# sony/DiffRoll

Measured on AMD Instinct MI355X. Metric: piano-roll frames/sec (200-step sample), higher is better.
Workload: dtype f32

## Files before the change

diffroll_amd/csrc/abi.hip:

```cpp
#include "engine_state.h"
#include "tenants.h"

#include <algorithm>
#include <condition_variable>
#include <mutex>

namespace drh {

thread_local std::string g_create_error;
void release_stager(int dev);
std::atomic<int> g_engines[MAX_DEVICES];

struct FusedSlot {
    std::mutex mu;
    std::condition_variable cv;
    dr_engine* owner = nullptr;
    bool claimed = false;
    hipEvent_t done = nullptr;
};
FusedSlot g_slots[MAX_DEVICES];

bool claim_fused_slot(dr_engine* e, hipStream_t st) {
    FusedSlot& s = g_slots[e->cfg.device];
    std::unique_lock<std::mutex> lk(s.mu);
// ... 367 lines not shown
        (void)hipDeviceSynchronize();
        e->opt.solver = value;
        e->hist_key.valid = false;
        if (!e->committed) return DR_OK;
        return build_solver(e);
    }
    if (n == "solver_noise") {
        if (value != 0 && value != 1)
            return fail(e, DR_EINVAL, "solver_noise is 0 (the deterministic solver) or 1 (its stochastic form, SDE-DPM-Solver++), got %d", value);
        if (e->opt.solver_noise == value) return DR_OK;
        if (e->opt.solver != 0) (void)hipDeviceSynchronize();
        e->opt.solver_noise = value;
        e->hist_key.valid = false;
        if (!e->committed || e->opt.solver == 0) return DR_OK;
        return build_solver(e);
    }
    if (n == "start_step") {
        if (value < -1 || value >= e->S)
            return fail(e, DR_EINVAL, "start_step is -1 (the chain's first step) or in [0, timesteps = %d), got %d", e->S, value);
        e->opt.start = value;
        return DR_OK;
    }
    if (n == "start_noise") {
        if (value != 0 && value != 1)
            return fail(e, DR_EINVAL, "start_noise is 0 (x on entry is x at the start step) or 1 (a clean roll, diffused to it), got %d", value);
        e->opt.start_noise = value;
        return DR_OK;
    }
    if (n == "x0_clip") {
        if (value < 0 || value > 2)
            return fail(e, DR_EINVAL, "x0_clip is 0 (off), 1 (clamp the x0 prediction to [0, 1]) or 2 (to [-1, 1]), got %d", value);
        if (e->opt.x0_clamp != value) e->hist_key.valid = false;
        e->opt.x0_clamp = value;
        return DR_OK;
    }
    if (n == "x0_threshold") {
        if (value != 0 && (value < 5000 || value > 10000))
            return fail(e, DR_EINVAL, "x0_threshold is 0 (off) or the percentile in units of 1 / 10000, 5000 .. 10000 (9950 = 99.5 %%), got %d", value);
        if (e->opt.x0_thresh != value) e->hist_key.valid = false;
        e->opt.x0_thresh = value;
        return DR_OK;
    }
    if (n == "guidance_t_min" || n == "guidance_t_max") {
        const bool is_max = n == "guidance_t_max";
        if (!guidance_value_ok(is_max, value, e->S))
            return fail(e, DR_EINVAL, is_max ? "guidance_t_max is -1 (= timesteps - 1) or in [0, timesteps = %d), got %d"
                                             : "guidance_t_min is in [0, timesteps = %d), got %d", e->S, value);
        (is_max ? e->opt.guid.hi : e->opt.guid.lo) = value;
        return DR_OK;
    }
    if (!lab) return fail(e, DR_ENAME, "unknown option '%s'", name);
    if (n == "fused_stack_xcd") { if (e->opt_stack_xcd != value) drop(); e->opt_stack_xcd = value; return DR_OK; }
    if (n == "fused_stack_warm") { if (e->opt_stack_warm != value) drop(); e->opt_stack_warm = value; return DR_OK; }
#ifdef DR_FAULT_HOOK
    if (n == "stack_fault_test") { if (e->opt_stack_fault != value) drop(); e->opt_stack_fault = value; return DR_OK; }
#endif
    if (n == "stack_ticks") { if (e->stack_dbg_on != value) drop(); e->stack_dbg_on = value; return DR_OK; }
    if (n.compare(0, 5, "tune.") == 0) {
        Tuning& t = tuning();
        const std::string f = n.substr(5);
        if (f == "ksplit_blocks") {
            if (t.ksplit_blocks.load() != value) { t.ksplit_blocks.store(value); tuning_epoch().fetch_add(1); drop(); }
            return DR_OK;
        }
        std::atomic<int>* field = f == "pack_threads" ? &t.pack_threads : f == "tile" ? &t.tile : f == "pw" ? &t.pw : f == "pw_nw" ? &t.pw_nw
                   : f == "pwk" ? &t.pwk : f == "ksplit_max" ? &t.ksplit_max : f == "one_ks" ? &t.one_ks : f == "stack3" ? &t.stack3
                   : f == "stack_fl" ? &t.stack_fl : f == "tail_t4" ? &t.tail_t4 : f == "xcd_n" ? &t.xcd_n : f == "xcd_model" ? &t.xcd_model
                   : f == "s3_eager" ? &t.s3_eager : f == "debug_chunks" ? &t.debug_chunks : nullptr;
        if (!field) return fail(e, DR_ENAME, "unknown option '%s'", name);
        if (field->load() != value) {
            field->store(value);
            tuning_epoch().fetch_add(1);
            drop();
        }
        return DR_OK;
    }
    return fail(e, DR_ENAME, "unknown option '%s'", name);
}

int open_chain_call(dr_engine* e, int sampler, int B, int T, const int* step, int& NB, int& i0, hipStream_t st) {
    int rc = check_ready(e, sampler, B, T);
    if (rc) return rc;
    if (step) {
        const int t = *step;
        if (t < 0 || t >= e->S) return fail(e, DR_EINVAL, "step %d out of range", t);
        if (!e->rs_steps.empty() && std::find(e->rs_steps.begin(), e->rs_steps.end(), t) == e->rs_steps.end())
            return fail(e, DR_EINVAL, "step %d is not visited by the respaced chain (option sampling_steps = %d)", t, e->opt.steps);
    }
    if ((rc = check_options(e, sampler, B, NB, T))) return rc;
    i0 = 0;
    if (!step && (rc = start_position(e, i0))) return rc;
    if ((rc = ensure_workspace(e, NB, T))) return rc;
    if (e->opt.solver == 2) {
        const size_t need = 2 * (size_t)B * T * 88;
        if (!e->hist.fits(need)) e->hist_key.valid = false;
        if ((rc = grow_chain_buffer(e, e->hist, need, st))) return rc;
    }
    if (e->opt.x0_thresh != 0 && (rc = grow_chain_buffer(e, e->thresh_work, thresh_work_words(B), st))) return rc;
    return DR_OK;
}

}
using namespace drh;

extern "C" {

// ... 483 lines not shown
```

diffroll_amd/csrc/engine_state.h:

```cpp
#pragma once
#include <hip/hip_runtime.h>

#include <dlfcn.h>

#include <atomic>
#include <chrono>
#include <cmath>
#include <cstdarg>
#include <cstdio>
#include <cstdlib>
#include <cstring>
#include <map>
#include <memory>
#include <string>
#include <thread>
#include <vector>

#include "../../include/diffroll_amd_debug.h"
#include "device_buffer.h"
#include "fused_mode.h"
#include "kernels.h"

namespace drh {
using namespace dr;
// ... 95 lines not shown
    dr_config cfg{};
    int C = 0, Cp = 0, L = 0, K = 0, S = 0, NM = 0;
    int max_dil = 1;
    int n_bins = 0, bins_p = 0;
    std::string err;
    std::map<std::string, std::vector<float>> params;
    std::vector<float> h_emb, h_coef;
    std::vector<float> h_win, h_fb;
    float h_win_norm = 0.f;
    bool committed = false;

    drh::DevBuf<float> d_coef;
    drh::DevBuf<float> d_dtab;
    std::vector<drh::LayerW> layers;
    float *in_w = nullptr, *in_b = nullptr, *skip_w = nullptr, *skip_b = nullptr, *outp_w = nullptr, *outp_b = nullptr;
    float *dft_w = nullptr, *mel_w = nullptr;
    float *fft_win = nullptr, *fft_tw = nullptr;
    float fft_norm = 1.f;
    bool use_fft = false;
    std::vector<drh::DevBuf<float>> consts;

    int ws_NB = 0, ws_T = 0;
    drh::DevBuf<float> sk_ws;
    drh::DevBuf<unsigned> sk_cnt;
    drh::DevBuf<float> h, hd, g, skip, tmp, x0buf;
    drh::DevBuf<float> xwork;
    drh::DevBuf<float> hd3, g3;
    int prec = 0;
    bool s3_ready = false;
    double t_pack_s = 0.0, t_upload_s = 0.0, t_tables_s = 0.0, t_capture_s = 0.0;
    int norm_framewise = 0;
    int fe_B = 0, fe_T = 0;
    drh::DevBuf<float> cond;
    drh::DevBuf<float> cond_dummy;
    drh::DevBuf<float> cond_tr;
    int cond_tr_T = 0;
    drh::DevBuf<float> wav_pad, power, logmel, specP4, mm;

    drh::GraphKey gkey;
    hipGraph_t graph = nullptr;
    hipGraphExec_t gexec = nullptr;
    drh::DevBuf<long long> dbg_ticks;
    drh::DevBuf<unsigned long long> d_counts;
    size_t mm_scratch_off = 0;
    hipStream_t cap_stream = nullptr;
    drh::DevBuf<dr::DynParams> d_dyn;
    drh::DevBuf<int> d_tsel;
    bool use_dyn = false;

    drh::FusedMode fused;
    int opt_stack_xcd = 1;
    int opt_stack_fault = 0;
    int opt_stack_warm = 0;
    int n_cus = 0;
    drh::StackSync sync;
    int opt_tail = 1;
    int64_t tail_launches = 0;
    drh::ChainOptions opt;
    std::vector<int> win_marks;
    drh::DevBuf<unsigned> d_wintab;
    std::vector<int> rs_steps;
    drh::DevBuf<float> d_coef_rs;
    std::vector<float> h_solver;
    drh::DevBuf<float> d_solver;
    drh::DevBuf<float> hist;
    int hist_par = 0;
    struct { bool valid = false; int sampler = -1, B = 0, T = 0, t = -1; } hist_key;
    drh::DevBuf<unsigned> thresh_work;
    int64_t inproj_launches = 0;
    int64_t conv0_launches = 0;
    unsigned win_epoch = 0;
    drh::DevBuf<float> xalt;
    int last_mode = 0;
    unsigned tuning_epoch = 0;
    long kfd_gpu_id = -1;
    double last_tenant_scan_s = -1.0;
    hipStream_t graph_stream = nullptr;
    bool graph_stream_set = false;
    bool unverified = false;
    hipStream_t fused_stream = nullptr;
    int opt_blocked = 2;
    drh::DevBuf<float> xsave;
    drh::DevBuf<long long> stack_dbg;
    int stack_dbg_on = 0;
    int64_t stack_launches = 0;

    double prof_flops = 0.0;
    std::string prof_name;
    bool prof = false;
    std::vector<std::pair<hipEvent_t, hipEvent_t>> prof_events;
    size_t prof_used = 0;
    int64_t prof_launches = 0;
    double prof_ms = 0.0;

    ~dr_engine() {
        if (gexec) (void)hipGraphExecDestroy(gexec);
        if (graph) (void)hipGraphDestroy(graph);
        if (cap_stream) (void)hipStreamDestroy(cap_stream);
        for (auto& p : prof_events) { (void)hipEventDestroy(p.first); (void)hipEventDestroy(p.second); }
    }
};

namespace drh {

inline int fail(dr_engine* e, int code, const char* fmt, ...) {
    char buf[512];
// ... 103 lines not shown
```

diffroll_amd/csrc/gemm_body.h:

```cpp
#pragma once
#include "device_common.h"

namespace dr {

DR_DEVINL void residual_quad(const float (&v)[4], const float4 bias, const float4 prev, float (&o)[4]) {
    float bb[4], pv[4];
    f4arr(bias, bb); f4arr(prev, pv);
#pragma unroll
    for (int e = 0; e < 4; ++e) o[e] = div_sqrt2(pv[e] + (v[e] + bb[e]));
}
DR_DEVINL void skip_quad(const float (&v)[4], const float4 bias, const float4 prev, const bool skip_init, float (&o)[4]) {
    float bb[4], pv[4];
    f4arr(bias, bb); f4arr(prev, pv);
#pragma unroll
    for (int e = 0; e < 4; ++e) o[e] = skip_init ? v[e] + bb[e] : (v[e] + bb[e]) + pv[e];
}
DR_DEVINL long cond_row(const GemmArgs& a, const int b) {
    int r = a.c_b0 + b;
    if (a.c_n > 0 && r >= a.c_n) r %= a.c_n;
    return r;
}
DR_DEVINL void gate_quad(const float (&v0)[4], const float (&v1)[4], const float4 bias0, const float4 bias1,
                         const float4 cond0, const float4 cond1, const bool has_c, float (&o)[4]) {
    float b0[4], b1[4], c0[4], c1[4];
// ... 473 lines not shown
    #pragma unroll
                        for (int e = 0; e < 4; ++e) o[e] = v0[e] * v0[e] + v1[e] * v1[e];
                    }
                    if (a.out_s3 & 1) {
                        store_s3_quad<COH>(a.Y + (long)be * a.y_bs, o, c0, t, a.T, a.y_rows >> 3, a.wt_store);
                    } else {
                        float* dst = a.Y + (long)be * a.y_bs + (long)(c0 >> 2) * a.y_ps + (long)t * a.y_fs;
                        store_f4<COH>(dst, make_float4(o[0], o[1], o[2], o[3]), a.wt_store);
                    }
                } else {
                    const int p0 = mt * 128 + wave * 32 + rq;
                    float v[4], o[4];
    #pragma unroll
                    for (int e = 0; e < 4; ++e) v[e] = acc[ni][4 * q + e];
                    if constexpr (EPI == EPI_RES_SKIP) {
                        if (p0 < a.y_rows) {
                            float* dst = a.Y + (long)be * a.y_bs + (long)(p0 >> 2) * a.y_ps + (long)t * a.y_fs;
                            residual_quad(v, ebias[q], eop[ni][q], o);
                            *reinterpret_cast<float4*>(dst) = make_float4(o[0], o[1], o[2], o[3]);
                            if (a.Y2) store_y2<COH, 0>(a, be, o, ed2[q], p0, t);
                        } else {
                            float* dst = a.skip + (long)be * a.s_bs + ((long)((p0 - a.y_rows) >> 2) * a.T + t) * 4;
                            skip_quad(v, ebias[q], eop[ni][q], a.skip_init, o);
                            *reinterpret_cast<float4*>(dst) = make_float4(o[0], o[1], o[2], o[3]);
                        }
                    } else {
                        if (p0 >= a.y_rows) continue;
                        float bb[4];
                        f4arr(ebias[q], bb);
    #pragma unroll
                        for (int e = 0; e < 4; ++e) {
                            if constexpr (EPI == EPI_PLAIN) o[e] = a.alpha * v[e] + bb[e];
                            else if constexpr (EPI == EPI_RELU) o[e] = fmaxf(a.alpha * v[e] + bb[e], 0.f);
                            else if constexpr (EPI == EPI_SILU) { const float z = v[e] + bb[e]; o[e] = z * sigmoidf_(z); }
                            else o[e] = logf(v[e] + 1e-6f);
                        }
                        float* dst = a.Y + (long)be * a.y_bs + (long)(p0 >> 2) * a.y_ps + (long)t * a.y_fs;
                        *reinterpret_cast<float4*>(dst) = make_float4(o[0], o[1], o[2], o[3]);
                        if constexpr (EPI == EPI_RELU) {
                            if (a.Y2) store_y2<COH, 0>(a, be, o, ed2[q], p0, t);
                        }
                    }
                }
            }
        }
    }
    if (a.dbg && blockIdx.x == 0 && tid == 0) {
        a.dbg[0] = tick1 - tick0;
        a.dbg[1] = clock64() - tick0;
    }
}

template <int NW, int COH, int RLDS, int TBN = 32 * NW, int EPI = EPI_RES_SKIP>
DR_DEVINL void pw_body(const GemmArgs& a, const int mt, const int nt, const int wave, float4* Rs = nullptr, const int foff = 0) {
    static_assert(EPI == EPI_RES_SKIP || EPI == EPI_RELU || EPI == EPI_PLAIN, "pw_body epilogues");
    static_assert(EPI == EPI_RES_SKIP || !RLDS, "the LDS-resident tile belongs to the residual / skip epilogue");
    constexpr int BN = TBN;
    int lane = threadIdx.x & 63;
    if constexpr (COH) asm volatile("" : "+v"(lane));
    const int r = lane & 31, hi = lane >> 5;
    const long long tick0 = a.dbg ? clock64() : 0;

    const int tps = (a.T + BN - 1) / BN;
    const int b = nt / tps;
    const int t0 = (nt % tps) * BN + foff;
    const int NS = a.kchunks;

    const __amdgpu_buffer_rsrc_t wr = __builtin_amdgcn_make_buffer_rsrc(
        (void*)(a.Wp + (long)mt * NS * 4096), 0, (unsigned)NS * 16384u, 0x00020000);
    const __amdgpu_buffer_rsrc_t xr = __builtin_amdgcn_make_buffer_rsrc(
        (void*)(a.X + (long)b * a.x_bs), 0, (unsigned)(a.x_planes * a.x_ps * 4), 0x00020000);
    const int wvo = (hi * 128 + wave * 32 + r) * 16;
    const int xps = (int)a.x_ps * 4;
    int xvo[NW];
#pragma unroll
    for (int ni = 0; ni < NW; ++ni) xvo[ni] = hi * xps + min(t0 + ni * 32 + r, a.T - 1) * 16;

    struct BF { float4 v[4][NW]; };
    auto load_a = [&](int slab) { return load_a4(wr, wvo, slab, NS, 120); };
    auto load_b = [&](int slab) -> BF {
        BF o;
#pragma unroll
        for (int g = 0; g < 4; ++g)
#pragma unroll
            for (int ni = 0; ni < NW; ++ni)
                o.v[g][ni] = buffer_load_f4(xr, xvo[ni], (slab * 8 + g * 2) * xps);
        return o;
    };

    f32x16 acc[NW];
#pragma unroll
    for (int ni = 0; ni < NW; ++ni)
#pragma unroll
        for (int e = 0; e < 16; ++e) acc[ni][e] = 0.f;

    AF4 aA = load_a(0), aB;
    BF bA = load_b(0), bB;
    auto step = [&](auto ROLE, int slab) {
        constexpr bool kB = decltype(ROLE)::value;
        const int nxt = min(slab + 1, NS - 1);
        if constexpr (kB) { aA = load_a(nxt); bA = load_b(nxt); }
        else { aB = load_a(nxt); bB = load_b(nxt); }
#pragma unroll
        for (int g = 0; g < 4; ++g) {
            const float4 af = kB ? aB.v[g] : aA.v[g];
#pragma unroll
            for (int ni = 0; ni < NW; ++ni) acc[ni] = __builtin_amdgcn_mfma_f32_32x32x2f32(af.x, (kB ? bB.v[g][ni] : bA.v[g][ni]).x, acc[ni], 0, 0, 0);
// ... 22 lines not shown
        const float* base = res_rows ? a.Y + (long)b * a.y_bs + (long)(rowb >> 2) * a.y_ps
                                     : a.skip + (long)b * a.s_bs + (long)((rowb - a.y_rows) >> 2) * a.T * 4;
        const long qs = res_rows ? 2 * a.y_ps : (long)2 * a.T * 4;
        const long fs = res_rows ? a.y_fs : 4;
#pragma unroll
        for (int ni = 0; ni < NW; ++ni) {
            const int tc = min(t0 + ni * 32 + r, a.T - 1);
#pragma unroll
            for (int q = 0; q < 4; ++q) eop[ni][q] = *reinterpret_cast<const float4*>(base + q * qs + tc * fs);
        }
    };
    int slab = 0;
    const int pre = max(NS - 2, 0) & ~1;
    for (; slab < pre; slab += 2) {
        step(std::false_type{}, slab);
        step(std::true_type{}, slab + 1);
        if (a.dbg && slab == 0 && blockIdx.x == 0 && threadIdx.x == 0) a.dbg[2] = clock64() - tick0;
    }
    if (a.dbg && blockIdx.x == 0 && threadIdx.x == 0) a.dbg[3] = clock64() - tick0;
    if constexpr (!RLDS) load_epilogue();
    __builtin_amdgcn_sched_barrier(0);
    for (; slab + 2 <= NS; slab += 2) {
        step(std::false_type{}, slab);
        step(std::true_type{}, slab + 1);
    }
    if (slab < NS) step(std::false_type{}, slab);
    const long long tick1 = a.dbg ? clock64() : 0;
    if constexpr (RLDS) load_epilogue();

#pragma unroll
    for (int ni = 0; ni < NW; ++ni) {
        const int t = t0 + ni * 32 + r;
        if (t >= a.T) continue;
#pragma unroll
        for (int q = 0; q < 4; ++q) {
            const int p0 = rowb + 8 * q;
            float v[4], o[4];
#pragma unroll
            for (int e = 0; e < 4; ++e) v[e] = acc[ni][4 * q + e];
            if constexpr (EPI != EPI_RES_SKIP) {
                if (p0 >= a.y_rows) continue;
                float bb[4];
                f4arr(ebias[q], bb);
#pragma unroll
                for (int e = 0; e < 4; ++e) {
                    o[e] = a.alpha * v[e] + bb[e];
                    if constexpr (EPI == EPI_RELU) o[e] = fmaxf(o[e], 0.f);
                }
                float* dst = a.Y + (long)b * a.y_bs + (long)(p0 >> 2) * a.y_ps + (long)t * a.y_fs;
                store_f4<COH>(dst, make_float4(o[0], o[1], o[2], o[3]), a.wt_store);
                continue;
            }
            float4* rs = nullptr;
            if constexpr (RLDS) rs = Rs + (wave * 8 + 2 * q + hi) * BN + foff + ni * 32 + r;
#ifdef DR_BOUNDS
            if constexpr (RLDS) DR_CHECK_LDS(rs, lds_off(Rs), lds_off(Rs) + 32u * BN * 16u, 121);
#endif
            float4 pv;
            if constexpr (RLDS) pv = *rs;
            else pv = eop[ni][q];
            if (res_rows) {
                float* dst = a.Y + (long)b * a.y_bs + (long)(p0 >> 2) * a.y_ps + (long)t * a.y_fs;
                residual_quad(v, ebias[q], pv, o);
                if constexpr (RLDS) *rs = make_float4(o[0], o[1], o[2], o[3]);
                else *reinterpret_cast<float4*>(dst) = make_float4(o[0], o[1], o[2], o[3]);
                if (a.Y2) store_y2<0, COH>(a, b, o, ed2[q], p0, t);
            } else {
                float* dst = a.skip + (long)b * a.s_bs + ((long)((p0 - a.y_rows) >> 2) * a.T + t) * 4;
                skip_quad(v, ebias[q], pv, a.skip_init, o);
                if constexpr (RLDS) *rs = make_float4(o[0], o[1], o[2], o[3]);
                else *reinterpret_cast<float4*>(dst) = make_float4(o[0], o[1], o[2], o[3]);
            }
        }
    }
    if (a.dbg && blockIdx.x == 0 && threadIdx.x == 0) {
        a.dbg[0] = tick1 - tick0;
        a.dbg[1] = clock64() - tick0;
    }
}

template <int NJ, int KS, int EPI>
DR_DEVINL void gemm16_body(const GemmArgs& a, char* smem, const int mt, const int nt) {
    static_assert(EPI == EPI_GATE || EPI == EPI_RES_SKIP, "16x16 variant: hot kernels only");
    constexpr int BN = 32 * NJ;
    constexpr int XP = 8 * KS;
    constexpr int RT = 2;
    constexpr int CT = 2 * NJ;

    const int tid = threadIdx.x;
    const int lane = tid & 63;
    const int wave = __builtin_amdgcn_readfirstlane(tid >> 6);
    const int halo = ((a.taps - 1) >> 1) * a.dil;
    const int FW = BN + 2 * halo;
    float4* Xs = reinterpret_cast<float4*>(smem);
    float4* Rs = Xs + 2 * XP * FW;
#ifdef DR_BOUNDS
    const unsigned xs0 = lds_off(Xs), xs1 = xs0 + 2u * XP * FW * 16u, rs1 = xs1 + (EPI == EPI_RES_SKIP ? 32u * BN * 16u : 0u);
    if (tid == 0) DR_CHECK(rs1 <= (unsigned)a.lds_bytes, 140, rs1, a.lds_bytes);
#endif

    const int tps = (a.T + BN - 1) / BN;
    const int b = nt / tps;
    const int t0 = (nt % tps) * BN;
    const int NS = a.kchunks * a.taps;
    const int nchunks = a.kchunks / KS;

    if (wave >= 4) {
// ... 159 lines not shown
```

diffroll_amd/csrc/kernels.h:

```cpp
#pragma once
#include <hip/hip_runtime.h>
#include <stdint.h>

#include <atomic>

#include "launch_plan.h"

namespace dr {


struct Tuning {
    std::atomic<int> pack_threads{16};
    std::atomic<int> tile{0};
    std::atomic<int> pw{1};
    std::atomic<int> pw_nw{0};
    std::atomic<int> pwk{1};
    std::atomic<int> ksplit_max{16};
    std::atomic<long> ksplit_blocks{0};
    std::atomic<int> one_ks{0};
    std::atomic<int> stack3{1};
    std::atomic<int> stack_fl{0};
    std::atomic<int> tail_t4{0};
    std::atomic<int> xcd_n{-1};
    std::atomic<int> xcd_model{1};
// ... 29 lines not shown
    int y_rows;
    const float* cond;
    long c_bs;
    int c_b0, c_n;
    const float* cond2;
    int n_cond;
    int dual;
    float* skip;
    long s_bs;
    int skip_init;
    float alpha;
    int xcd_n;
    float* ws;
    unsigned* ws_cnt;
    size_t ws_floats, ws_cnt_n;
    int ksplit;
    long long* dbg;
    int lds_bytes;
    int fold128;
    int nofold64;
    int wt_store;
};

hipError_t init_kernels();
hipError_t read_bounds(unsigned long long* out4);
hipError_t reset_bounds();
hipError_t launch_gemm(const GemmArgs& a, int epi, int NI, hipStream_t s, int prec = 0);
hipError_t launch_gemm16(const GemmArgs& a, int epi, int NJ, hipStream_t s);
hipError_t launch_pointwise(const GemmArgs& a, int NW, hipStream_t s);
hipError_t launch_pointwise_ksplit(const GemmArgs& a, int NW, hipStream_t s);

struct StackLayer {
    const float *conv_w, *conv_b, *conv_b2;
    const float *cond, *cond2;
    const float *out_w, *out_b;
    int dil, pad_;
};
struct StackArgs {
    float *h, *hd, *g, *skip;
    const float* d2;
    const int* tsel;
    long d2_ts;
    const float* zero;
    int NB, T, Cp, taps, n_cond, L;
    long c_bs;
    int c_b0, c_n;
    int p0, p1;
    int xcd_n;
    int rs_off;
    int lds_bytes;
    int fault;
    int fold128;
    int warm;
    unsigned* xid;
    unsigned* bar;
    unsigned* err;
    unsigned* derr;
    long long* dbg;
    StackLayer layer[DR_STACK_MAX_LAYERS];
};
hipError_t launch_stack(const StackArgs& s, int FL, int max_dil, hipStream_t st, int prec = 0);

struct DynParams {
    unsigned long long seed;
    int first_sample;
    float w, onepw;
    unsigned epoch;
};
hipError_t launch_set_dyn(DynParams* d, unsigned long long seed, int first_sample, float w, float onepw, unsigned epoch,
                          hipStream_t s);

struct UpdateArgs {
    float* x;
    const float* x0c;
    const float* x0u;
    const float* noise;
    const float* coef;
    int t;
    int mode;
    long n;
    long per_sample;
    float w, onepw;
    uint64_t seed;
    int first_sample;
    const DynParams* dyn;
    int win;
    const unsigned* win_tab;
    int draw_n, draw_G;
    float* hist;
    int hist_par;
    float clamp_lo, clamp_hi;
};
__host__ __device__ inline const float* hist_prev(const UpdateArgs& a) { return a.hist + (a.hist_par ? a.n : 0); }
__host__ __device__ inline float* hist_next(const UpdateArgs& a) { return a.hist && a.t > 0 ? a.hist + (a.hist_par ? 0 : a.n) : nullptr; }
constexpr int WIN_BLEND_SHIFT = 28;
__host__ __device__ inline int win_H(const UpdateArgs& a) { return a.win & ((1 << WIN_BLEND_SHIFT) - 1); }
__host__ __device__ inline int win_blend(const UpdateArgs& a) { return a.win >> WIN_BLEND_SHIFT; }
constexpr unsigned window_entry(unsigned rec, unsigned idx) { return (rec << 16) | idx; }
constexpr int window_rec(unsigned w) { return (int)(w >> 16); }
constexpr int window_idx(unsigned w) { return (int)(w & 0xFFFFu); }
struct WindowTable { unsigned w[STACK_GROUPS]; };
hipError_t launch_set_windows(unsigned* d_tab, const WindowTable& tab, int n, hipStream_t s);
hipError_t launch_update(const UpdateArgs& a, hipStream_t s);
hipError_t launch_diffuse(const UpdateArgs& a, hipStream_t s);

constexpr int THRESH_HEAD = 4, THRESH_ROW_WORDS = 272, THRESH_SEL = 256, THRESH_QS = 264;
// ... 67 lines not shown
```

diffroll_amd/csrc/launch_plan.h:

```cpp
#pragma once
#include <algorithm>
#include <cstddef>

#include "../../include/diffroll_amd.h"

namespace dr {

enum Epilogue : int {
    EPI_PLAIN = 0,
    EPI_RELU = 1,
    EPI_SILU = 2,
    EPI_GATE = 3,
    EPI_RES_SKIP = 4,
    EPI_POWER = 5,
    EPI_LOG = 6
};

constexpr int DR_STACK_MAX_LAYERS = 30;
constexpr int STACK_GROUPS = 512;
constexpr size_t SK_WS_FLOATS = (size_t)16 << 20, SK_CNT_N = 4096;

struct PlanKnobs {
    int tile = 0, pw = 1, pw_nw = 0, pwk = 1, ksplit_max = 16;
    long ksplit_blocks = 0;
    int stack3 = 1, stack_fl = 0;
};

inline int gemm_block_frames(int NI) { return (NI == 3 || NI == 5) ? 32 * NI : 64 * NI; }
inline size_t gemm_lds_bytes(int NI, int KS, int taps, int dil, int prec, int epi) {
    const int halo = ((taps - 1) / 2) * dil;
    const int BN = gemm_block_frames(NI);
    const int FW = BN + 2 * halo;
    return (size_t)2 * (prec ? 12 : 8) * KS * FW * 16 + (epi == EPI_RES_SKIP ? (size_t)32 * BN * 16 : 0);
}

struct KSplitPlan { int ks; double us; double us_unsplit; };
inline KSplitPlan plan_ksplit(const PlanKnobs& k, long tiles, int nchunks, int kchunks, int taps, int NI, int prec,
                              size_t ws_floats, size_t ws_cnt_n) {
    const int ks_max = k.ksplit_max;
    const long forced_blocks = k.ksplit_blocks;
    const long max_blocks = forced_blocks ? forced_blocks : (prec ? 256 : 2048);
    const int BN = gemm_block_frames(NI);
    const double t_full = (double)kchunks * taps * 16.0 * (BN / 32) * 69.0 / 2400.0;
    auto cost = [&](int ks) {
        return (double)((tiles * ks + 255) / 256) * t_full / ks + (ks > 1 ? 4.0 + ks : 0.0);
    };
    KSplitPlan p{1, cost(1), cost(1)};
    for (int ks = 2; ks <= ks_max && ks <= 16; ks *= 2) {
        if (tiles * ks > max_blocks || nchunks % ks != 0) break;
        if ((size_t)tiles * ks * 128 * BN > ws_floats || (size_t)tiles * 4 > ws_cnt_n) break;
        const double c = cost(ks);
        if (tiles * ks <= 256 || c < 0.97 * p.us) { p.us = std::min(p.us, c); p.ks = ks; }
    }
    return p;
}

inline int stack_tile_frames(int FL) { return FL == 5 ? 160 : 64 * FL; }
inline size_t stack3_lds_bytes(int FL, int taps, int max_dil) {
    return std::max(gemm_lds_bytes(FL, 1, taps, max_dil, 1, EPI_GATE), gemm_lds_bytes(1, 4, 1, 1, 1, EPI_RES_SKIP)) + 16;
}
inline int stack_group_blocks(int FL, int Cp, int T) {
    const int BN = stack_tile_frames(FL);
    return (Cp >> 6) * ((T + BN - 1) / BN);
}
inline size_t stack_lds_bytes(int FL, int taps, int max_dil) {
    const int BN = stack_tile_frames(FL), halo = ((taps - 1) / 2) * max_dil;
    return (size_t)2 * 8 * (BN + 2 * halo) * 16 + (size_t)32 * BN * 16 + 16;
}

struct Tile { int flavor, n; };

inline double split_cost(const PlanKnobs& k, long blocks, int bn, double pen, int MT, int taps) {
    const int nchunks = 2 * MT;
    const KSplitPlan p = plan_ksplit(k, blocks, nchunks, nchunks, taps, bn / 64, 0, SK_WS_FLOATS, SK_CNT_N);
    if (p.ks <= 1 || blocks * p.ks <= 256) return 1e30;
    const double us_per_frame = p.us_unsplit / ((double)((blocks + 255) / 256) * bn);
    return 1.05 * pen * p.us / us_per_frame;
}
inline Tile pick_tile(const PlanKnobs& k, int MT, int NB, int T, int taps, int dil, int prec, int epi, bool allow16,
                      bool wide32 = false) {
    const int forced = k.tile;
    const int halo = ((taps - 1) / 2) * dil;
    struct Cand { int flavor, n, bn; double pen; };
    const Cand cands[] = {{0, 2, 128, 1.0}, {0, 5, 160, 1.04}, {1, 5, 160, 1.04}, {0, 3, 96, 1.04}, {1, 3, 96, 1.04}, {0, 1, 64, 1.0}};
    auto feasible = [&](const Cand& c) {
        if (c.flavor == 1 && (!allow16 || prec != 0)) return false;
        if (c.flavor == 0 && (c.n == 3 || c.n == 5) && (!wide32 || prec != 0 || epi != EPI_GATE || taps == 1)) return false;
        const int ks = (taps == 1) ? 2 : 1;
        const size_t lds = (c.flavor == 0)
            ? gemm_lds_bytes(c.n, (taps == 1 && c.n == 1) ? 4 : ks, taps, dil, prec, epi)
            : (size_t)2 * 8 * ks * (c.bn + 2 * halo) * 16 + (epi == EPI_RES_SKIP ? (size_t)32 * c.bn * 16 : 0);
        return lds <= 160 * 1024;
    };
    if (forced) {
        const int ff = forced / 100 == 16 ? 1 : 0, fn = forced % 100;
        for (const Cand& c : cands)
            if (c.flavor == ff && c.n == fn && feasible(c)) return Tile{ff, fn};
    }
    Tile best{0, 1};
    double best_cost = 1e30;
    for (const Cand& c : cands) {
        if (!feasible(c)) continue;
        const long blocks = (long)MT * NB * ((T + c.bn - 1) / c.bn);
        double cost = (double)((blocks + 255) / 256) * c.bn * c.pen;
        if (c.flavor == 0 && c.n <= 2 && prec == 0 && epi == EPI_GATE && taps > 1 && allow16)
            cost = std::min(cost, split_cost(k, blocks, c.bn, c.pen, MT, taps));
        if (cost < best_cost - 1e-9) { best_cost = cost; best = Tile{c.flavor, c.n}; }
    }
    return best;
}
inline int pick_ni(const PlanKnobs& k, int MT, int NB, int T, int taps, int dil, int prec = 0) {
    return pick_tile(k, MT, NB, T, taps, dil, prec, EPI_GATE, false).n;
}
inline Tile pick_pointwise_tile(const PlanKnobs& k, int MT, int NB, int T, int prec, int kchunks = 0) {
    if (prec) return Tile{0, 1};
    const int pw = k.pw, pw_ni = k.pw_nw;
// ... 109 lines not shown
```

diffroll_amd/csrc/plan.hip:

```cpp
#include "engine_state.h"

namespace drh {

hipError_t launch_tiled(const GemmArgs& a, int epi, Tile t, hipStream_t s, int prec) {
    if (t.flavor == 3) return launch_pointwise_ksplit(a, t.n, s);
    if (t.flavor == 2) return launch_pointwise(a, t.n, s);
    return t.flavor == 1 ? launch_gemm16(a, epi, t.n, s) : launch_gemm(a, epi, t.n, s, prec);
}
void allow_splitk(const dr_engine* e, GemmArgs& a) {
    a.ws = e->sk_ws; a.ws_cnt = e->sk_cnt;
    a.ws_floats = SK_WS_FLOATS; a.ws_cnt_n = SK_CNT_N;
}

const float* g_zero_vecs[MAX_DEVICES] = {};
const float* zero_vec() {
    int dev = 0;
    (void)hipGetDevice(&dev);
    return (dev >= 0 && dev < MAX_DEVICES) ? g_zero_vecs[dev] : nullptr;
}

GemmArgs p4_gemm(const float* Wp, const float* bias, int MT, const float* X, int planes, int NB, int T) {
    GemmArgs a{};
    a.d2 = zero_vec();
    a.Wp = Wp; a.bias = bias ? bias : zero_vec(); a.MT = MT;
// ... 64 lines not shown
}

template <class Launch, class Account>
static int profiled(dr_engine* e, hipStream_t st, bool eligible, Launch&& launch, Account&& account) {
    const bool timed = e->prof && eligible && e->prof_used < e->prof_events.size();
    if (timed) HIPCHK(e, hipEventRecord(e->prof_events[e->prof_used].first, st));
    if (int rc = launch()) return rc;
    if (timed) {
        HIPCHK(e, hipEventRecord(e->prof_events[e->prof_used++].second, st));
        account();
    }
    return DR_OK;
}

static int launch_inproj(const Eval& v, const PlanKnobs& k) {
    dr_engine* e = v.e;
    const int Cp = e->Cp, T = v.T;
    const long act_bs = (long)Cp * T;
    GemmArgs a{};
    a.Wp = e->in_w; a.bias = e->in_b; a.MT = (Cp + 127) / 128;
    a.X = v.xin; a.x_bs = (long)T * 88; a.x_ps = 4; a.x_fs = 88; a.x_planes = 22; a.x_bmod = v.bmod;
    a.kchunks = 3; a.NB = v.NB; a.T = T; a.taps = 1; a.dil = 1; a.alpha = 1.f;
    p4_out(a, e->h, Cp / 4, T, Cp);
    a.d2 = e->d_dtab + (v.tsel ? 0 : (size_t)v.t * e->L * Cp);
    a.tsel = v.tsel; a.d2_ts = (long)e->L * Cp;
    if (e->prec) { a.Y2 = e->hd3; a.y2_bs = act_bs + act_bs / 2; a.out_s3 = 2; }
    else { a.Y2 = e->hd; a.y2_bs = act_bs; }
    allow_splitk(e, a);
    HIPCHK(e, launch_gemm(a, EPI_RELU, pick_ni(k, a.MT, v.NB, T, 1, 1), v.st));
    e->inproj_launches += 1;
    return DR_OK;
}

static int launch_stack_range(const Eval& v, const NetPlan& p, int p0, int p1) {
    dr_engine* e = v.e;
    const int Cp = e->Cp, L = e->L, T = v.T, prec = e->prec;
    const long act_n = (long)Cp * T, c_bs = (long)2 * Cp * T;
    int b0 = 0;
    for (int ck = 0; ck < p.stack_chunks; ++ck) {
        const int nb = v.NB / p.stack_chunks + (ck < v.NB % p.stack_chunks ? 1 : 0);
        StackArgs sa{};
        sa.h = e->h + b0 * act_n; sa.hd = e->hd + b0 * act_n; sa.g = e->g + b0 * act_n; sa.skip = e->skip + b0 * act_n;
        if (prec) { sa.hd = e->hd3 + b0 * (act_n + act_n / 2); sa.g = e->g3 + b0 * (act_n + act_n / 2); }
        sa.d2 = e->d_dtab + (v.tsel ? 0 : (size_t)v.t * L * Cp);
        sa.tsel = v.tsel ? v.tsel + b0 : nullptr; sa.d2_ts = (long)L * Cp;
        sa.zero = zero_vec();
        sa.NB = nb; sa.T = T; sa.Cp = Cp; sa.taps = e->K; sa.L = L;
        sa.n_cond = std::max(0, std::min(nb, v.n_cond - b0));
        sa.c_bs = c_bs;
        sa.c_b0 = b0 < v.n_cond ? b0 : 0; sa.c_n = e->fe_B;
        sa.p0 = p0; sa.p1 = p1;
        sa.xcd_n = e->opt_stack_xcd;
        sa.warm = e->opt_stack_warm;
        sa.fault = e->opt_stack_fault;
        sa.fold128 = e->opt_blocked >= 2;
        sa.bar = e->sync.bar(); sa.err = e->sync.err; sa.derr = e->sync.derr(); sa.xid = e->sync.xid();
        sa.dbg = e->stack_dbg_on ? e->stack_dbg : nullptr;
        for (int l = 0; l < L; ++l) {
            const LayerW& w = e->layers[l];
            StackLayer& y = sa.layer[l];
            y.conv_w = prec ? w.conv_w3 : w.conv_w; y.conv_b = w.conv_b;
            y.conv_b2 = v.zero_spec ? w.conv_b_z : w.conv_b_u;
            y.cond2 = nullptr;
            if (e->cond_tr && !v.zero_spec) { y.cond2 = e->cond_tr + (size_t)l * 2 * Cp * T; y.conv_b2 = w.conv_b; }
            y.cond = e->cond ? e->cond + (size_t)l * e->fe_B * 2 * Cp * T : e->cond_dummy;
            y.out_w = prec ? w.out_w3 : w.out_w; y.out_b = w.out_b; y.dil = w.dil;
        }
        int rc = profiled(e, v.st, true, [&]() -> int {
            HIPCHK(e, launch_stack(sa, p.stack_fl, e->max_dil, v.st, prec));
            e->stack_launches += 1;
            e->unverified = true; e->fused_stream = v.st;
            return DR_OK;
        }, [&] {
            const double C = e->C, fr = (double)nb * T;
            for (int q = p0; q < p1; ++q)
                e->prof_flops += fr * 2.0 * C * 2.0 * C * ((q & 1) ? (q == 2 * L - 1 ? 0.5 : 1.0) : (double)e->K);
            e->prof_name = "stack_kernel<" + std::to_string(p.stack_fl) + "> (fused residual stack: dilated conv k=" +
                           std::to_string(e->K) + " + conditioner + gate and 1x1 + residual/skip, phases " +
                           std::to_string(p0) + ".." + std::to_string(p1 - 1) + " of " + std::to_string(2 * L) +
                           (p.stack_chunks > 1 ? ", " + std::to_string(p.stack_chunks) + " sample chunks" : "") +
                           (prec ? (p.fold ? ", split-bf16, blocked accumulation" : ", split-bf16, one chain per output")
                                 : (p.fold ? ", blocked accumulation" : ", one fp32 chain per output")) + ")";
        });
        if (rc) return rc;
        b0 += nb;
    }
    return DR_OK;
}

static int launch_conv(const Eval& v, const NetPlan& p, const PlanKnobs& k, int l) {
    dr_engine* e = v.e;
    const int Cp = e->Cp, L = e->L, T = v.T, NB = v.NB, bmod = v.bmod, prec = e->prec;
    const LayerW& w = e->layers[l];
    GemmArgs a = p4_gemm(prec ? w.conv_w3 : w.conv_w, w.conv_b, Cp / 64, e->hd, Cp / 4, NB, T);
    if (prec) s3_in(a, e->hd3, Cp, T);
    a.bias2 = v.zero_spec ? w.conv_b_z : w.conv_b_u;
    if (e->cond_tr && !v.zero_spec) {
        a.cond2 = e->cond_tr + (size_t)l * 2 * Cp * T;
        a.bias2 = w.conv_b;
    }
    a.taps = e->K; a.dil = w.dil;
    a.fold128 = e->opt_blocked >= 2;
    a.cond = e->cond ? e->cond + (size_t)l * e->fe_B * 2 * Cp * T : e->cond_dummy;
    a.c_bs = (long)2 * Cp * T;
    a.c_n = e->fe_B;
    a.n_cond = v.n_cond;
// ... 236 lines not shown
```

diffroll_amd/csrc/stack.hip:

```cpp
#include "gemm_body.h"
#include "persistent.h"

namespace dr {

DR_BOUNDS_TU(stack)

template <int FL, int FOLDP = 1, int PREC = 0>
__global__ __launch_bounds__(512) void stack_kernel(const StackArgs s_by_value) {
    extern __shared__ __attribute__((aligned(16))) char smem[];
    (void)s_by_value;
    typedef const __attribute__((address_space(4))) StackArgs* KernArgs;
    const KernArgs sp = (KernArgs)__builtin_amdgcn_kernarg_segment_ptr();
    const __attribute__((address_space(4))) StackArgs& s = *sp;
    static_assert(FL == 1 || FL == 2 || (FL == 5 && FOLDP == 1 && PREC == 0), "block flavours");
    constexpr int BN = FL == 5 ? 160 : 64 * FL;
    constexpr int RP = 32;
    constexpr int RWL = (BN + 63) / 64;
    const int wave = __builtin_amdgcn_readfirstlane(threadIdx.x >> 6);
    const int MT = s.Cp >> 6;
    const int MB = MT;
    const int tps = (s.T + BN - 1) / BN;
    const unsigned gsize = (unsigned)(MB * tps);
    int mt, nt, grp, member;
    if (s.xcd_n) {
        const int xcd = blockIdx.x & 7, idx = blockIdx.x >> 3;
        member = idx % (int)gsize;
        grp = (idx / (int)gsize) * 8 + xcd;
    } else {
        member = blockIdx.x % (int)gsize;
        grp = blockIdx.x / (int)gsize;
    }
    if (grp >= s.NB) return;
    mt = member % MB;
    nt = grp * tps + member / MB;
    const unsigned pending_timeout = __hip_atomic_load(s.derr, __ATOMIC_RELAXED, __HIP_MEMORY_SCOPE_AGENT);
    DR_CHECK(grp >= 0 && grp < 512 && (long)grp * gsize + member < 1024, 130, grp, member);
    unsigned* ctr = s.bar + 4 * grp;
    const long act_bs = (long)s.Cp * s.T;
    const int P = s.Cp >> 2;
    unsigned episode = 0;
    float4* Rs = reinterpret_cast<float4*>(smem + s.rs_off);
    const int b_ = nt / tps, t0_ = (nt % tps) * BN;
    auto tile_plane = [&](int pl, bool& is_res) -> float* {
        const int row0 = mt * 128 + pl * 4;
        is_res = row0 < s.Cp;
        return is_res ? s.h + (long)b_ * act_bs + (long)(row0 >> 2) * s.T * 4
                      : s.skip + (long)b_ * act_bs + (long)((row0 - s.Cp) >> 2) * s.T * 4;
    };
    if constexpr (PREC) {
        if (pending_timeout) return;
    } else {
#ifdef DR_BOUNDS
        if (threadIdx.x == 0) DR_CHECK(s.rs_off + RP * BN * 16 + 16 <= s.lds_bytes && lds_off(smem) == 0u, 132, s.rs_off, s.lds_bytes);
#endif
        dma_tile<BN, 0>(Rs, [&](int pl) { bool is_res; return tile_plane(pl, is_res); }, s.T, t0_, wave, 8, threadIdx.x & 63, 131);
        if (pending_timeout) return;
        if (s.p0 & 1) {
            asm volatile("s_waitcnt vmcnt(0)" ::: "memory");
            __syncthreads();
        }
    }
    int wt_store = 1;
    unsigned my_tag = 0;
    unsigned& same_xcd_s = *reinterpret_cast<unsigned*>(Rs + RP * BN);
    if (threadIdx.x == 0) {
        unsigned my_xcc;
        asm volatile("s_getreg_b32 %0, hwreg(HW_REG_XCC_ID)" : "=s"(my_xcc));
        const unsigned gen = __hip_atomic_fetch_add(ctr + 2, 0u, __ATOMIC_RELAXED, __HIP_MEMORY_SCOPE_AGENT);
        my_tag = (gen << 4) | (my_xcc & 0xfu);
        __hip_atomic_store(s.xid + (long)grp * gsize + member, my_tag, __ATOMIC_RELAXED, __HIP_MEMORY_SCOPE_AGENT);
    }

#pragma unroll 1
    for (int p = s.p0; p < s.p1; ++p) {
        const int l = p >> 1;
        const __attribute__((address_space(4))) StackLayer& ly = sp->layer[l];
        if (s.dbg && blockIdx.x == 0 && threadIdx.x == 0) {
            s.dbg[p - s.p0] = clock64();
            if (p == s.p0) s.dbg[120] = wall_clock64();
        }
        GemmArgs a{};
        a.d2 = s.zero;
        a.lds_bytes = s.lds_bytes;
        a.wt_store = wt_store;
        a.MT = MT; a.NB = s.NB; a.T = s.T; a.alpha = 1.f; a.ksplit = 1;
        a.x_bs = act_bs; a.x_ps = (long)s.T * 4; a.x_fs = 4; a.x_planes = P; a.kchunks = s.Cp >> 5;
        a.y_bs = act_bs; a.y_ps = (long)s.T * 4; a.y_fs = 4; a.y_rows = s.Cp;
        if constexpr (PREC) {
            const long s3_bs = act_bs + act_bs / 2;
            if ((p & 1) == 0) {
                a.Wp = ly.conv_w; a.bias = ly.conv_b; a.bias2 = ly.conv_b2;
                a.X = s.hd; a.x_bs = s3_bs; a.x_piece = (long)(s.Cp >> 3) * s.T * 4; a.x_planes = s.Cp >> 3;
                a.taps = s.taps; a.dil = ly.dil;
                a.cond = ly.cond; a.cond2 = ly.cond2; a.c_bs = s.c_bs; a.c_b0 = s.c_b0; a.c_n = s.c_n; a.n_cond = s.n_cond;
                a.Y = s.g; a.y_bs = s3_bs; a.out_s3 = 1;
                gemm_body<FL, 1, EPI_GATE, 1, 1, FOLDP>(a, smem, mt, nt, 0);
            } else {
                a.Wp = ly.out_w; a.bias = ly.out_b;
                a.X = s.g; a.x_bs = s3_bs; a.x_piece = (long)(s.Cp >> 3) * s.T * 4; a.x_planes = s.Cp >> 3;
                a.taps = 1; a.dil = 1;
                a.Y = s.h;
                const bool last = (l + 1 == s.L);
                if (!last) {
                    a.Y2 = s.hd; a.y2_bs = s3_bs; a.out_s3 = 2;
                    a.d2 = s.d2 + (long)(l + 1) * s.Cp; a.tsel = s.tsel; a.d2_ts = s.d2_ts;
                }
                a.skip = s.skip; a.s_bs = act_bs; a.skip_init = (l == 0);
                const bool idle = last && mt < (s.Cp >> 7);
                const int tps64 = (s.T + 63) >> 6;
                const int b_ = nt / tps, ti = nt % tps;
#pragma unroll 1
                for (int half = 0; half < BN / 64; ++half) {
                    const int t64 = ti * (BN / 64) + half;
                    if (half) {
                        asm volatile("s_waitcnt vmcnt(0)" ::: "memory");
                        __syncthreads();
                    }
                    if (!idle && t64 < tps64) gemm_body<1, 4, EPI_RES_SKIP, 1, 1>(a, smem, mt, b_ * tps64 + t64, 0);
                }
            }
        } else
        if ((p & 1) == 0) {
            a.Wp = ly.conv_w; a.bias = ly.conv_b; a.bias2 = ly.conv_b2;
            a.X = s.hd; a.taps = s.taps; a.dil = ly.dil;
            a.cond = ly.cond; a.cond2 = ly.cond2; a.c_bs = s.c_bs; a.c_b0 = s.c_b0; a.c_n = s.c_n; a.n_cond = s.n_cond;
            a.Y = s.g;
            if (s.dbg && p + 2 >= s.p1) a.dbg = s.dbg + 64;
            gemm_body<FL, 1, EPI_GATE, 0, 1, FOLDP>(a, smem, mt, nt, 0);
            if (wave == 4) __builtin_amdgcn_fence(__ATOMIC_ACQUIRE, "agent");
            if (wave >= 4 && s.warm) {
                const int be = nt / tps;
                if (be < s.n_cond)
                    l2_touch(ly.cond + cond_row(a, be) * s.c_bs + (long)mt * 32 * s.T * 4, (unsigned)(32 * s.T * 16), wave - 4, 4);
                l2_touch(ly.out_w + (long)mt * (s.Cp >> 5) * 4096, (unsigned)((s.Cp >> 5) * 16384), wave - 4, 4);
            }
        } else {
            a.Wp = ly.out_w; a.bias = ly.out_b;
            a.X = s.g; a.taps = 1; a.dil = 1;
            a.Y = s.h;
            const bool last = (l + 1 == s.L);
            if (!last) {
                a.Y2 = s.hd; a.y2_bs = act_bs;
                a.d2 = s.d2 + (long)(l + 1) * s.Cp; a.tsel = s.tsel; a.d2_ts = s.d2_ts;
            }
            a.skip = s.skip; a.s_bs = act_bs; a.skip_init = (l == 0);
            const bool idle = last && mt < (s.Cp >> 7);
            if (s.dbg && p + 3 == s.p1) a.dbg = s.dbg + 96;
            if constexpr (FL == 2) {
                if (!idle) pw_body<2, 1, 1, 128>(a, mt, nt, wave & 3, Rs, (wave >> 2) * 64);
            } else if constexpr (FL == 5) {
                if (!idle) {
                    if (wave < 4) pw_body<3, 1, 1, 160>(a, mt, nt, wave, Rs, 0);
                    else pw_body<2, 1, 1, 160>(a, mt, nt, wave - 4, Rs, 96);
                }
            } else {
                if (wave < 4 && !idle) pw_body<BN / 32, 1, 1>(a, mt, nt, wave, Rs);
            }
            if (wave >= 4 && s.warm && !last) {
                const __attribute__((address_space(4))) StackLayer& nx = sp->layer[l + 1];
                l2_touch(nx.conv_w + (long)mt * (s.Cp >> 5) * s.taps * 4096, (unsigned)(2 * s.taps * 16384), wave - 4, 4);
            }
        }
        if (p + 1 < s.p1) {
            group_barrier<false>(ctr, ++episode * (gsize + DR_FAULT_EXTRA(s)), s.err, s.derr);
            if (episode == 1) {
                if (threadIdx.x == 0) {
                    unsigned same = 1;
                    for (unsigned i = 0; i < gsize; ++i)
                        same &= (__hip_atomic_load(s.xid + (long)grp * gsize + i, __ATOMIC_RELAXED, __HIP_MEMORY_SCOPE_AGENT) == my_tag);
                    same_xcd_s = same;
                }
                __syncthreads();
                wt_store = __builtin_amdgcn_readfirstlane(same_xcd_s ? 0 : 1);
            }
        }
    }
    if (s.dbg && blockIdx.x == 0 && threadIdx.x == 0) {
        s.dbg[s.p1 - s.p0] = clock64();
        s.dbg[121] = wall_clock64();
    }
    if constexpr (!PREC) {
        asm volatile("s_waitcnt vmcnt(0)" ::: "memory");
        __syncthreads();
        const int lane = threadIdx.x & 63;
        for (int i = wave; i < RP * RWL; i += 8) {
            const int pl = i / RWL, seg = i - pl * RWL;
            bool is_res;
            float* dst = tile_plane(pl, is_res);
            const int t = t0_ + seg * 64 + lane;
#ifdef DR_BOUNDS
            if (seg * 64 + lane < BN) DR_CHECK_LDS(Rs + pl * BN + seg * 64 + lane, s.rs_off, s.rs_off + RP * BN * 16, 133);
#endif
            if (seg * 64 + lane < BN && t < s.T && (!is_res || s.p1 < 2 * s.L))
                *reinterpret_cast<float4*>(dst + (long)t * 4) = Rs[pl * BN + seg * 64 + lane];
        }
    }
    if (threadIdx.x == 0) {
        const unsigned left = __hip_atomic_fetch_add(ctr + 1, 1u, __ATOMIC_RELAXED, __HIP_MEMORY_SCOPE_AGENT);
        if (left == gsize - 1) {
            __hip_atomic_store(ctr, 0u, __ATOMIC_RELAXED, __HIP_MEMORY_SCOPE_AGENT);
            __hip_atomic_store(ctr + 1, 0u, __ATOMIC_RELAXED, __HIP_MEMORY_SCOPE_AGENT);
            __hip_atomic_fetch_add(ctr + 2, 1u, __ATOMIC_RELAXED, __HIP_MEMORY_SCOPE_AGENT);
        }
    }
}

hipError_t launch_stack(const StackArgs& s, int FL, int max_dil, hipStream_t st, int prec) {
    if (FL != 1 && FL != 2 && FL != 5) return hipErrorInvalidValue;
    if (prec && ((s.Cp & 127) || FL == 5)) return hipErrorInvalidValue;
    if (s.L < 1 || s.L > DR_STACK_MAX_LAYERS || s.p0 < 0 || s.p1 > 2 * s.L || s.p0 >= s.p1 || (s.Cp & 63)) return hipErrorInvalidValue;
    const int BN = stack_tile_frames(FL), MT = s.Cp >> 6, gsize = stack_group_blocks(FL, s.Cp, s.T);
// ... 42 lines not shown
```

Before: 2265.

## Split fused-stack output projection into residual and skip row slabs per block

In the fused FL=2 stack path, each block now handles a 64-row residual slab and a 64-row skip slab of the output projection rather than a contiguous 128-row tile. The LDS residual tile and the L2 prefetch of output weights follow the new slab mapping. On the last layer only the skip slab is computed, so every block has work instead of half sitting idle. It is on by default through a new option and adds a second weight-tile prefetch per block, and it drops the next-layer conv-weight warmup on this path.

```diff
diff --git a/diffroll_amd/csrc/abi.hip b/diffroll_amd/csrc/abi.hip
--- a/diffroll_amd/csrc/abi.hip
+++ b/diffroll_amd/csrc/abi.hip
@@ -443,6 +443,7 @@
     if (!lab) return fail(e, DR_ENAME, "unknown option '%s'", name);
     if (n == "fused_stack_xcd") { if (e->opt_stack_xcd != value) drop(); e->opt_stack_xcd = value; return DR_OK; }
     if (n == "fused_stack_warm") { if (e->opt_stack_warm != value) drop(); e->opt_stack_warm = value; return DR_OK; }
+    if (n == "fused_stack_defer") { if (e->opt_stack_slabs != value) drop(); e->opt_stack_slabs = value != 0; return DR_OK; }
 #ifdef DR_FAULT_HOOK
     if (n == "stack_fault_test") { if (e->opt_stack_fault != value) drop(); e->opt_stack_fault = value; return DR_OK; }
 #endif
diff --git a/diffroll_amd/csrc/engine_state.h b/diffroll_amd/csrc/engine_state.h
--- a/diffroll_amd/csrc/engine_state.h
+++ b/diffroll_amd/csrc/engine_state.h
@@ -171,6 +171,7 @@
     int opt_stack_xcd = 1;
     int opt_stack_fault = 0;
     int opt_stack_warm = 0;
+    int opt_stack_slabs = 1;
     int n_cus = 0;
     drh::StackSync sync;
     int opt_tail = 1;
diff --git a/diffroll_amd/csrc/gemm_body.h b/diffroll_amd/csrc/gemm_body.h
--- a/diffroll_amd/csrc/gemm_body.h
+++ b/diffroll_amd/csrc/gemm_body.h
@@ -549,7 +549,7 @@
 }
 
 template <int NW, int COH, int RLDS, int TBN = 32 * NW, int EPI = EPI_RES_SKIP>
-DR_DEVINL void pw_body(const GemmArgs& a, const int mt, const int nt, const int wave, float4* Rs = nullptr, const int foff = 0) {
+DR_DEVINL void pw_body(const GemmArgs& a, const int mt, const int nt, const int wave, float4* Rs = nullptr, const int foff = 0, const int slot = -1) {
     static_assert(EPI == EPI_RES_SKIP || EPI == EPI_RELU || EPI == EPI_PLAIN, "pw_body epilogues");
     static_assert(EPI == EPI_RES_SKIP || !RLDS, "the LDS-resident tile belongs to the residual / skip epilogue");
     constexpr int BN = TBN;
@@ -678,7 +678,7 @@
                 continue;
             }
             float4* rs = nullptr;
-            if constexpr (RLDS) rs = Rs + (wave * 8 + 2 * q + hi) * BN + foff + ni * 32 + r;
+            if constexpr (RLDS) rs = Rs + ((slot < 0 ? wave : slot) * 8 + 2 * q + hi) * BN + foff + ni * 32 + r;
 #ifdef DR_BOUNDS
             if constexpr (RLDS) DR_CHECK_LDS(rs, lds_off(Rs), lds_off(Rs) + 32u * BN * 16u, 121);
 #endif
diff --git a/diffroll_amd/csrc/kernels.h b/diffroll_amd/csrc/kernels.h
--- a/diffroll_amd/csrc/kernels.h
+++ b/diffroll_amd/csrc/kernels.h
@@ -105,6 +105,7 @@
     int fault;
     int fold128;
     int warm;
+    int slabs;
     unsigned* xid;
     unsigned* bar;
     unsigned* err;
diff --git a/diffroll_amd/csrc/launch_plan.h b/diffroll_amd/csrc/launch_plan.h
--- a/diffroll_amd/csrc/launch_plan.h
+++ b/diffroll_amd/csrc/launch_plan.h
@@ -62,6 +62,16 @@
 inline int stack_group_blocks(int FL, int Cp, int T) {
     const int BN = stack_tile_frames(FL);
     return (Cp >> 6) * ((T + BN - 1) / BN);
+}
+#ifdef __HIPCC__
+#define DR_PLAN_HD __host__ __device__
+#else
+#define DR_PLAN_HD
+#endif
+struct StackSlab { int row0, tile, half; };
+DR_PLAN_HD inline StackSlab stack_slab(int Cp, int m, bool skip) {
+    const int row0 = (skip ? Cp : 0) + 64 * m;
+    return StackSlab{row0, row0 >> 7, (row0 >> 6) & 1};
 }
 inline size_t stack_lds_bytes(int FL, int taps, int max_dil) {
     const int BN = stack_tile_frames(FL), halo = ((taps - 1) / 2) * max_dil;
diff --git a/diffroll_amd/csrc/plan.hip b/diffroll_amd/csrc/plan.hip
--- a/diffroll_amd/csrc/plan.hip
+++ b/diffroll_amd/csrc/plan.hip
@@ -140,6 +140,7 @@
         sa.p0 = p0; sa.p1 = p1;
         sa.xcd_n = e->opt_stack_xcd;
         sa.warm = e->opt_stack_warm;
+        sa.slabs = (p.stack_fl == 2 && !prec) ? e->opt_stack_slabs : 0;
         sa.fault = e->opt_stack_fault;
         sa.fold128 = e->opt_blocked >= 2;
         sa.bar = e->sync.bar(); sa.err = e->sync.err; sa.derr = e->sync.derr(); sa.xid = e->sync.xid();
diff --git a/diffroll_amd/csrc/stack.hip b/diffroll_amd/csrc/stack.hip
--- a/diffroll_amd/csrc/stack.hip
+++ b/diffroll_amd/csrc/stack.hip
@@ -39,10 +39,12 @@
     const long act_bs = (long)s.Cp * s.T;
     const int P = s.Cp >> 2;
     unsigned episode = 0;
+    const bool slabs = FL == 2 && PREC == 0 && s.slabs;
+    const StackSlab res_slab = stack_slab(s.Cp, mt, false), skip_slab = stack_slab(s.Cp, mt, true);
     float4* Rs = reinterpret_cast<float4*>(smem + s.rs_off);
     const int b_ = nt / tps, t0_ = (nt % tps) * BN;
     auto tile_plane = [&](int pl, bool& is_res) -> float* {
-        const int row0 = mt * 128 + pl * 4;
+        const int row0 = slabs ? (pl < 16 ? res_slab.row0 + pl * 4 : skip_slab.row0 + (pl - 16) * 4) : mt * 128 + pl * 4;
         is_res = row0 < s.Cp;
         return is_res ? s.h + (long)b_ * act_bs + (long)(row0 >> 2) * s.T * 4
                       : s.skip + (long)b_ * act_bs + (long)((row0 - s.Cp) >> 2) * s.T * 4;
@@ -132,7 +134,8 @@
                 const int be = nt / tps;
                 if (be < s.n_cond)
                     l2_touch(ly.cond + cond_row(a, be) * s.c_bs + (long)mt * 32 * s.T * 4, (unsigned)(32 * s.T * 16), wave - 4, 4);
-                l2_touch(ly.out_w + (long)mt * (s.Cp >> 5) * 4096, (unsigned)((s.Cp >> 5) * 16384), wave - 4, 4);
+                l2_touch(ly.out_w + (long)(slabs ? res_slab.tile : mt) * (s.Cp >> 5) * 4096, (unsigned)((s.Cp >> 5) * 16384), wave - 4, 4);
+                if (slabs) l2_touch(ly.out_w + (long)skip_slab.tile * (s.Cp >> 5) * 4096, (unsigned)((s.Cp >> 5) * 16384), wave - 4, 4);
             }
         } else {
             a.Wp = ly.out_w; a.bias = ly.out_b;
@@ -147,7 +150,12 @@
             const bool idle = last && mt < (s.Cp >> 7);
             if (s.dbg && p + 3 == s.p1) a.dbg = s.dbg + 96;
             if constexpr (FL == 2) {
-                if (!idle) pw_body<2, 1, 1, 128>(a, mt, nt, wave & 3, Rs, (wave >> 2) * 64);
+                if (slabs && !last) {
+                    const StackSlab& sl = wave < 4 ? res_slab : skip_slab;
+                    pw_body<2, 1, 1, 128>(a, sl.tile, nt, 2 * sl.half + (wave & 1), Rs, ((wave >> 1) & 1) * 64, (wave < 4 ? 0 : 2) + (wave & 1));
+                } else if (slabs) {
+                    pw_body<1, 1, 1, 128>(a, skip_slab.tile, nt, 2 * skip_slab.half + (wave & 1), Rs, (wave >> 1) * 32, 2 + (wave & 1));
+                } else if (!idle) pw_body<2, 1, 1, 128>(a, mt, nt, wave & 3, Rs, (wave >> 2) * 64);
             } else if constexpr (FL == 5) {
                 if (!idle) {
                     if (wave < 4) pw_body<3, 1, 1, 160>(a, mt, nt, wave, Rs, 0);
@@ -156,7 +164,7 @@
             } else {
                 if (wave < 4 && !idle) pw_body<BN / 32, 1, 1>(a, mt, nt, wave, Rs);
             }
-            if (wave >= 4 && s.warm && !last) {
+            if (wave >= 4 && s.warm && !last && !slabs) {
                 const __attribute__((address_space(4))) StackLayer& nx = sp->layer[l + 1];
                 l2_touch(nx.conv_w + (long)mt * (s.Cp >> 5) * s.taps * 4096, (unsigned)(2 * s.taps * 16384), wave - 4, 4);
             }
```

Result: no change. 2275 (median of 6 runs) (+0.4%).
